# LSimon95/megatts2

Measured on AMD Instinct MI355X. Metric: mel-frames/sec (whole node), higher is better.
Workload: dtype f32; 1 GPU; C3: B=32/GPU x 1 GPU, Np=70, Tp=431, Tm=431; stages vqpe+mrte+adm+plm+decoder+vocoder; forced durations; weights=synthetic (name-seeded), parallelism=dp1 (utterance shards, one RCCL all-gather of mels per step)

## Files before the change

### include/megatts2_hip.h

```cpp
#ifndef MEGATTS2_HIP_H
#define MEGATTS2_HIP_H

#include <stddef.h>
#include <stdint.h>

#ifdef __cplusplus
extern "C" {
#endif

typedef struct mt2_model mt2_model;

typedef struct mt2_config {
    int32_t mel_bins, mrte_hidden, mrte_kernel, mrte_stride, mrte_n_layer, mrte_n_stack, mrte_n_block;
    int32_t content_ff_dim, content_n_heads, content_n_layers, phone_vocab;
    int32_t vq_mel_bins, vq_stride, vq_hidden, vq_kernel, vq_n_layers, vq_n_stacks, vq_n_blocks, vq_bins, vq_dim;
    int32_t dec_kernel, dec_hidden, dec_n_stack, dec_n_block;
    int32_t plm_layers, plm_heads, plm_vq_dim, plm_tc_dim, plm_bins;
    int32_t adm_layers, adm_heads, adm_emb_dim, adm_tc_dim, adm_tc_emb_dim;
    int32_t hg_in_dim, hg_init_channels, hg_n_up, hg_up_rates[8], hg_up_kernels[8];
    int32_t hg_n_res, hg_res_kernels[4], hg_res_dilations[4][3];
    float hg_slope;
    int32_t max_positions;
    int32_t hg_inference_padding;
    int32_t hg_reflect_pad;
// ... 243 lines not shown
} mt2_attn_desc;
int mt2_op_attention_desc(void* stream, const mt2_attn_desc* d);
int mt2_attention_route(const mt2_attn_desc* d, int32_t* err, int32_t* kernel, int32_t* tmpl, int32_t* launch, long long* lds);
int mt2_gemm_trace_begin(mt2_model* m);
int mt2_gemm_trace_end(mt2_model* m, int cap, const char** names, int64_t* launches, double* flops, double* ms);
int mt2_gemm_trace_shapes(mt2_model* m, char* buf, int cap, int top);
int mt2_gemm_config_count(void);
const char* mt2_gemm_config_name(int idx);
int mt2_gemm_route(int M, int N, int K, int taps, int dil, int groups, int pro_act, int operands, int misaligned, int force_cfg,
                   int x3h, int* err, int* cfg, int* variant, long long* lds, int* planes);
int mt2_conv_pair_route(int R, int C, int taps, int dil, int flags, int pair_fuse, int x3h, int* err, long long* lds, int* grid,
                        int* block, int* bm, int* bmo);
int mt2_op_conv_pair(void* stream, const float* X, int ldx, int R, int C, int taps, int dil, float slope, const void* Wh1,
                     const float* inv1, const float* bias1, const void* Wh2, const float* inv2, const float* bias2,
                     const int32_t* valid, float* Y, int ldy, int pair_fuse, int32_t* range_flag);
int mt2_op_gemm_x3h_ln(void* stream, const float* X, int ldx, int Rx, int a_mul, int shift0, const float* W, const void* W3,
                       const void* Wh, const float* wh_inv, const float* bias, const float* R, int ldr, float* C, int ldc, int M, int N,
                       int K, int epi_act, int force_cfg, float* stat_out, int32_t* stat_nt, int32_t* stat_w, const float* ln_stat,
                       int ln_nt, int ln_w, const float* ln_s, float ln_eps);
int mt2_bench_gemm(void* stream, int M, int N, int K, int taps, int dil, int flags, int force_cfg, int iters,
                   int w_copies, float* avg_ms, char* cfg_name, int cfg_name_cap, double* sustained_ghz);

#ifdef __cplusplus
}
#endif
#endif
```

### megatts2_amd/csrc/capi.inc

```

#include <climits>

namespace mt2 {
extern thread_local std::string g_last_error;
void finalize_model(mt2_model& m);
}

using namespace mt2;

#define MT2_API_BEGIN try {
#define MT2_API_END                                 \
    ::CallScope::verdict_of_open_call();            \
    return 0;                                       \
    }                                               \
    catch (const std::exception& e) {               \
        g_last_error = e.what();                    \
        return -1;                                  \
    }                                               \
    catch (...) {                                   \
        g_last_error = "unknown error";             \
        return -1;                                  \
    }

enum Need { NEED_G = 1, NEED_ADM = 2, NEED_PLM = 4, NEED_VOC = 8 };
// ... 257 lines not shown
    if (n == "t_x6_128") return &m->opts.t_x6_128;
    if (n == "t_x3h_128") return &m->opts.t_x3h_128;
    if (n == "x3h") return &m->opts.x3h;
    if (n == "x6_ks") return &m->opts.x6_ks;
    if (n == "voc_streams") return &m->opts.voc_streams;
    if (n == "ldr_prio") return &m->opts.ldr_prio;
    if (n == "skinny_rows") return &m->opts.skinny_rows;
    if (n == "skinny_nw") return &m->opts.skinny_nw;
    if (n == "skinny_pairs") return &m->opts.skinny_pairs;
    if (n == "attn_lds_min") return &m->opts.attn_lds_min;
    if (n == "attn_x6_min") return &m->opts.attn_x6_min;
    if (n == "ln_pairs_adm") return &m->opts.ln_pairs_adm;
    if (n == "ln_pairs_maxm") return &m->opts.ln_pairs_maxm;
    if (n == "a_planes") return &m->opts.a_planes;
    if (n == "pair_fuse") return &m->opts.pair_fuse;
    return nullptr;
}
static bool* option_flag(mt2_model* m, const std::string& n) {
    if (n == "splitk") return &m->opts.splitk;
    if (n == "stage_markers") return &m->opts.markers;
    if (n == "win_conv") return &m->opts.win_conv;
    if (n == "x6_conv") return &m->opts.x6_conv;
    if (n == "x6_gemm") return &m->opts.x6_gemm;
    if (n == "skinny_tm") return &m->opts.skinny_tm;
    if (n == "ldr64") return &m->opts.ldr64;
    return nullptr;
}
int mt2_set_option(mt2_model* m, const char* name, int value) {
    MT2_API_BEGIN
    MT2_REQUIRE(m != nullptr && name != nullptr, "null argument");
// ... 844 lines not shown
    return 0;
}
int mt2_op_conv_pair(void* stream, const float* X, int ldx, int R, int C, int taps, int dil, float slope, const void* Wh1,
                     const float* inv1, const float* bias1, const void* Wh2, const float* inv2, const float* bias2,
                     const int32_t* valid, float* Y, int ldy, int pair_fuse, int32_t* range_flag) {
    MT2_API_BEGIN
    PairP p{};
    p.X = X; p.ldx = ldx; p.R = R; p.C = C; p.taps = taps; p.dil = dil; p.slope = slope;
    p.Wh1 = Wh1; p.inv1 = inv1; p.bias1 = bias1; p.Wh2 = Wh2; p.inv2 = inv2; p.bias2 = bias2;
    p.wh_ldb = 4ll * (((long long)taps * C + 31) / 32 * 32);
    p.valid = valid; p.Y = Y; p.ldy = ldy;
    EngineOpts o;
    o.pair_fuse = pair_fuse;
    o.x3h_flag = range_flag;
    MT2_HIP(launch_conv_pair(p, (hipStream_t)stream, &o));
    MT2_API_END
}

int mt2_op_gemm(void* stream, const float* X, int ldx, int Rx, const int32_t* rowbase, int a_mul, int shift0,
                int taps, int dil, int Cin, const float* W, int ldw, const float* bias, const float* R, int ldr,
                const int32_t* valid, float* C, int ldc, int M, int N, int pro_act, float pro_slope, int epi_act,
                float out_scale, int force_cfg) {
    MT2_API_BEGIN
    GemmP p{};
    p.X = X; p.ldx = ldx; p.Rx = Rx; p.rowbase = rowbase; p.a_mul = a_mul ? a_mul : 1; p.shift0 = shift0;
    p.taps = taps; p.dil = dil; p.Cin = Cin; p.W = W; p.ldw = ldw; p.bias = bias; p.R = R; p.ldr = ldr;
    p.valid = valid; p.C = C; p.ldc = ldc; p.M = M; p.N = N; p.K = taps * Cin; p.groups = 1;
    p.pro_act = pro_act; p.pro_slope = pro_slope; p.epi_act = epi_act; p.out_scale = out_scale;
    EngineOpts o;
    o.force_cfg = force_cfg;
// ... 531 lines not shown
```

### megatts2_amd/csrc/gemm_x3h.hip

```cpp
#include "gemm_common.h"

#include <atomic>

#ifndef MT2_X3H_ABLATE
#define MT2_X3H_ABLATE 0
#endif
#define MT2_ABL_NOINGEST (MT2_X3H_ABLATE == 2 || MT2_X3H_ABLATE == 5 || MT2_X3H_ABLATE == 6 || MT2_X3H_ABLATE == 7)
#define MT2_ABL_NOSPLIT (MT2_X3H_ABLATE == 3 || MT2_X3H_ABLATE == 5 || MT2_X3H_ABLATE == 6)
#define MT2_ABL_NOBARRIER (MT2_X3H_ABLATE == 6 || MT2_X3H_ABLATE == 7)
#ifdef MT2_X3H_NO_BUFFER_LOADS
#define MT2_BUFFER_LOADS false
#else
#define MT2_BUFFER_LOADS true
#endif

namespace mt2 {

typedef _Float16 f16x8 __attribute__((ext_vector_type(8)));
typedef _Float16 f16x2 __attribute__((ext_vector_type(2)));
typedef float f32x2 __attribute__((ext_vector_type(2)));
typedef unsigned u32x4 __attribute__((ext_vector_type(4)));

constexpr float kX3hLoScale = 2048.0f, kX3hLoInv = 1.0f / 2048.0f, kX3hMaxIn = 65504.0f;

// ... 1376 lines not shown
    const EngineOpts& o = opts ? *opts : kDefaults;
    const PairRoute r = conv_pair_route(p_in, o);
    if (r.err != hipSuccess || r.grid == 0) return r.err;
    const PairTile& c = kPairTiles[r.tile];
    PairP p = p_in;
    p.x3h_flag = o.x3h_flag;
    p.ldr_prio = o.ldr_prio;
    const size_t lds_attr = c.ring + (size_t)(p.C / 32) * ((c.bm + 64 + 7) & ~7) * BK * sizeof(float);
    const hipError_t e = dyn_lds_once(g_pair_attr_done[r.tile], reinterpret_cast<const void*>(c.fn), lds_attr);
    if (e != hipSuccess) return e;
    if (opts) opts->last_cfg = "x3hpair";
    hipLaunchKernelGGL(c.fn, dim3(r.grid), dim3(r.block), r.lds, s, p);
    return hipGetLastError();
}


#define MT2_X3H_LDR(IDX_, BM_, BN_, WM_, WN_, NL_, NST_)                                                                    \
    { IDX_, BM_, BN_, (WM_* WN_ + NL_) * 64, (size_t)NST_ * ((size_t)BM_ * BK * 4 + (size_t)(2 * BN_ / 16) * 1024),         \
      "x3hldr" #BM_ "x" #BN_ "_" #WM_ "x" #WN_ "+" #NL_ "_s" #NST_ "xc",                                                    \
      { gemm_x3h_ldr_kernel<BM_, BN_, WM_, WN_, NL_, NST_, ACT_NONE>, gemm_x3h_ldr_kernel<BM_, BN_, WM_, WN_, NL_, NST_, ACT_RELU>, \
        gemm_x3h_ldr_kernel<BM_, BN_, WM_, WN_, NL_, NST_, ACT_LRELU>, gemm_x3h_ldr_kernel<BM_, BN_, WM_, WN_, NL_, NST_, PRO_APL>, \
        gemm_x3h_ldr_kernel<BM_, BN_, WM_, WN_, NL_, NST_, PRO_LNX> }, PIPE_X3H, 0, 0, (BN_) / (WN_) }
#define MT2_X3H_KS(IDX_, BM_, BN_, WM_, WN_, KS_, NL_, NST_)                                                                \
    { IDX_, BM_, BN_, (WM_* WN_ * KS_ + NL_) * 64, (size_t)KS_ * NST_ * ((size_t)BM_ * BK * 4 + (size_t)(2 * BN_ / 16) * 1024), \
      "x3hks" #BM_ "x" #BN_ "_" #WM_ "x" #WN_ "_k" #KS_ "+" #NL_ "_s" #NST_,                                                \
      { gemm_x3h_ks_kernel<BM_, BN_, WM_, WN_, KS_, NL_, NST_, ACT_NONE>, gemm_x3h_ks_kernel<BM_, BN_, WM_, WN_, KS_, NL_, NST_, ACT_RELU>, \
        gemm_x3h_ks_kernel<BM_, BN_, WM_, WN_, KS_, NL_, NST_, ACT_LRELU>, gemm_x3h_ks_kernel<BM_, BN_, WM_, WN_, KS_, NL_, NST_, PRO_APL>, \
        gemm_x3h_ks_kernel<BM_, BN_, WM_, WN_, KS_, NL_, NST_, PRO_LNX> }, PIPE_X3H, 0, KS_, 32 }
#define MT2_X3H_WIN(IDX_, QS_, BM_, BN_, WM_, WN_, NST_, NL_)                                                               \
    { IDX_, BM_, BN_, (WM_* WN_ + NL_) * 64, (size_t)NST_ * (((2 * BN_ / 16 + NL_ - 1) / NL_) * NL_ * 1024),                  \
// ... 17 lines not shown
```

### megatts2_amd/csrc/model_load.hip

```cpp
#include "mt2_model.h"
#include "x3h_planes.h"

#include <algorithm>
#include <cstring>

namespace mt2 {

thread_local std::string g_last_error;

void check_hip(hipError_t e, const char* what, const char* file, int line) {
    if (e != hipSuccess)
        throw Error(std::string("HIP error ") + hipGetErrorString(e) + " in " + what + " at " + file + ":" +
                    std::to_string(line));
}

Arena::~Arena() {
    for (auto& c : chunks_) (void)hipFree(c.p);
}
void Arena::reset() {
    for (auto& c : chunks_) c.used = 0;
}
void Arena::reserve(size_t bytes) {
    for (auto& c : chunks_)
        if (c.size >= bytes) return;
// ... 380 lines not shown
            for (int ph = 0; ph < hs; ++ph)
                for (int o = 0; o < co; ++o) {
                    float* rl = lo.data() + ((size_t)ph * co + o) * 2 * ch;
                    float* rh = hi.data() + ((size_t)ph * co + o) * 2 * ch;
                    for (int ci = 0; ci < ch; ++ci) {
                        rl[ci] = W(ci, o, ph + hs + s);
                        rl[ch + ci] = W(ci, o, ph + hs);
                        rh[ci] = W(ci, o, ph + s);
                        rh[ch + ci] = W(ci, o, ph);
                    }
                    bias[(size_t)ph * co + o] = b.data[o];
                }
            UpW u;
            u.cin = ch; u.cout = co; u.stride = s;
            u.wlo = L.upload(lo, (size_t)2 * ch); u.whi = L.upload(hi, (size_t)2 * ch); u.bias = L.upload(bias);
            m.hg_up.push_back(u);
            for (int j = 0; j < c.hg_n_res; ++j) {
                ResW r;
                r.k = c.hg_res_kernels[j];
                const std::string rp = "hifigan.resblocks." + std::to_string(i * c.hg_n_res + j);
                for (int n = 0; n < 3; ++n) {
                    r.dil[n] = c.hg_res_dilations[j][n];
                    r.c1[n] = L.conv(rp + ".convs1." + std::to_string(n), co, co, r.k);
                    r.c2[n] = L.conv(rp + ".convs2." + std::to_string(n), co, co, r.k);
                }
                m.hg_res.push_back(r);
            }
            ch = co;
        }
        m.hg_post = L.conv("hifigan.conv_post", 1, ch, 7);
// ... 12 lines not shown
```

### megatts2_amd/csrc/model_stages.hip

```cpp
#include "mt2_model.h"
#include "x3h_planes.h"
#include "gemm_tiles.h"

#include <algorithm>
#include <cmath>
#include <cstring>
#include <numeric>

namespace mt2 {



static RowSet make_rows(const int* lens, int B, int G) {
    RowSet rs;
    rs.B = B; rs.G = G;
    rs.len.assign(lens, lens + B);
    rs.off.resize(B);
    int r = G;
    for (int b = 0; b < B; ++b) {
        MT2_REQUIRE(lens[b] >= 0, "negative utterance length");
        rs.off[b] = r;
        r += lens[b] + G;
        rs.maxlen = std::max(rs.maxlen, lens[b]);
    }
// ... 175 lines not shown
                      bool reflect, float* y, const int* valid) {
    if (w1.k != w2.k || w1.cin != C || w1.cout != C || w2.cin != C || w2.cout != C) return false;
    GemmP g1{}, g2{};
    g1.W = w1.w; g1.taps = w1.k; g1.Cin = C; g1.groups = 1;
    g2.W = w2.w; g2.taps = w2.k; g2.Cin = C; g2.groups = 1;
    attach_planes(c.m, g1);
    attach_planes(c.m, g2);
    if (!g1.W3 || !g2.W3 || g1.wh_ldb != g2.wh_ldb) return false;
    PairP p{};
    p.X = x; p.ldx = C; p.R = R; p.C = C; p.taps = w1.k; p.dil = dil; p.slope = slope;
    p.Wh1 = g1.Wh; p.inv1 = g1.wh_inv; p.bias1 = w1.b;
    p.Wh2 = g2.Wh; p.inv2 = g2.wh_inv; p.bias2 = w2.b;
    p.wh_ldb = g1.wh_ldb ? g1.wh_ldb : 4ll * ((w1.k * C + 31) / 32 * 32);
    p.valid = valid; p.Y = y; p.ldy = C; p.reflect = reflect ? 1 : 0;
    const hipError_t e = launch_conv_pair(p, c.s, &c.m.opts);
    if (e == hipErrorNotSupported) return false;
    MT2_HIP(e);
    return true;
}

static void layernorm(const Ctx& c, const float* x, int ldx, const float* g, const float* b, int M, int C,
                      float* out, int ldo, const int* valid = nullptr, int valid_rows = 0,
                      const float* R1 = nullptr, int ldr1 = 0, int r1_rows = 0, int rows_per_group = 0,
                      int act = ACT_NONE, bool out_planes = false) {
    LnP p{};
    p.x = x; p.ldx = ldx; p.gamma = g; p.beta = b; p.rows_per_group = rows_per_group;
    p.R1 = R1; p.ldr1 = ldr1; p.r1_rows = r1_rows; p.valid = valid; p.valid_rows = valid_rows;
    p.out = out; p.ldo = ldo; p.M = M; p.C = C; p.eps = 1e-5f; p.act = act;
    p.out_planes = out_planes ? 1 : 0; p.x3h_flag = c.m.opts.x3h_flag;
    MT2_HIP(launch_layernorm(p, c.s));
// ... 965 lines not shown
    for (int b = 1; b < M0.B; ++b) min_len = std::min(min_len, M0.len[b]);
    auto halo = [&](const Ctx& cc, float* buf, int width, int G) {
        if (!reflect || G <= 0) return;
        MT2_REQUIRE(2ll * G <= (long long)M0.G * scale, "reflect padding needs a gap of two halos between utterances");
        MT2_REQUIRE((long long)min_len * scale > G, "reflect padding must be smaller than the utterance (as F.pad raises): "
                                                    "utterance too short for the vocoder's reflect-padded convolutions");
        MT2_HIP(launch_fill_reflect(buf, width, width, M0.d_start, M0.d_len, M0.B, scale, G, cc.s));
    };
    float* x = c.ws.get<float>((size_t)R * ch);
    if (reflect) {
        MT2_REQUIRE((cfg.hg_in_dim & 3) == 0, "reflect padding needs a mel width that is a multiple of 4");
        halo(c, const_cast<float*>(xmel), cfg.hg_in_dim, (m.hg_pre.k - 1) / 2);
    }
    conv_same(c, xmel, cfg.hg_in_dim, (int)R, m.hg_pre, x, ch, M0.d_valid);
    const int* valid = M0.d_valid;
    for (int i = 0; i < cfg.hg_n_up; ++i) {
        const UpW& u = m.hg_up[i];
        const int s = u.stride, co = u.cout, hs = s / 2;
        MT2_REQUIRE(R * s < (1ll << 31), "waveform row count exceeds int32");
        float* up = c.ws.get<float>((size_t)R * s * co);
        for (int half = 0; half < 2; ++half) {
            GemmP p{};
            p.X = x; p.ldx = ch; p.Rx = (int)R; p.taps = 2; p.shift0 = half == 0 ? -1 : 0; p.Cin = ch;
            p.W = half == 0 ? u.wlo : u.whi; p.bias = u.bias; p.valid = valid;
            p.C = up + (half == 0 ? 0 : hs * co); p.ldc = s * co; p.M = (int)R; p.N = hs * co;
            p.pro_act = ACT_LRELU; p.pro_slope = slope;
            gemm(c, p);
        }
        int* v2 = c.ws.get<int>((size_t)R * s);
        MT2_HIP(launch_expand_mask(valid, s, v2, R * s, c.s));
        valid = v2;
        R *= s;
        scale *= s;
        ch = co;
        const size_t per = (size_t)R * ch;
        float* rb[3] = {nullptr, nullptr, nullptr};
        MT2_REQUIRE(cfg.hg_n_res == 3, "HiFi-GAN V1 uses three resblocks per stage");
        const int nside = m.opts.voc_streams > 1 ? 2 : 0;
        ensure_aux(m, nside);
        if (reflect) {
            int g0 = 0;
            for (int j = 0; j < 3; ++j) g0 = std::max(g0, (m.hg_res[i * 3 + j].k - 1) / 2 * m.hg_res[i * 3 + j].dil[0]);
            halo(c, up, ch, g0);
        }
        if (nside) {
            MT2_HIP(hipEventRecord(m.ev_fork, c.s));
            m.aux_forked = true;
            for (int j = 0; j < nside; ++j) MT2_HIP(hipStreamWaitEvent(m.aux_streams[j], m.ev_fork, 0));
        }
        for (int j = 0; j < 3; ++j) {
            const ResW& r = m.hg_res[i * 3 + j];
// ... 14 lines not shown
                halo(cj, t1, ch, (r.k - 1) / 2);
                conv_same(cj, t1, ch, (int)R, r.c2[n], out, ch, valid, ACT_NONE, slope, ACT_NONE, h, ch, 1);
                h = out;
            }
        }
        for (int j = 0; j < nside; ++j) {
            MT2_HIP(hipEventRecord(m.ev_join[j], m.aux_streams[j]));
            MT2_HIP(hipStreamWaitEvent(c.s, m.ev_join[j], 0));
        }
        if (!reflect && i + 1 == cfg.hg_n_up && m.hg_post.cout == 1 && (ch & 3) == 0 && ch <= 128 && m.hg_post.k <= 15) {
            float* wav = c.ws.get<float>((size_t)R);
            const hipError_t e = launch_conv_post(rb[0], rb[1], rb[2], 1.0f / 3.0f, R, ch, m.hg_post.k, m.hg_post.w,
                                                  m.hg_post.b, 0.01f, valid, wav, c.s);
            if (e == hipSuccess) return wav;
            if (e != hipErrorNotSupported) MT2_HIP(e);
        }
        x = c.ws.get<float>(per);
        MT2_HIP(launch_avg3(rb[0], rb[1], rb[2], 1.0f / 3.0f, x, (long long)per, c.s));
    }
    float* wav = c.ws.get<float>((size_t)R);
    halo(c, x, ch, (m.hg_post.k - 1) / 2);
    conv_same(c, x, ch, (int)R, m.hg_post, wav, 1, valid, ACT_LRELU, 0.01f, ACT_TANH);
    return wav;
}


static double hz_to_mel_slaney(double f) {
    const double f_sp = 200.0 / 3.0, min_log_hz = 1000.0, min_log_mel = min_log_hz / f_sp, logstep = std::log(6.4) / 27.0;
    return f >= min_log_hz ? min_log_mel + std::log(f / min_log_hz) / logstep : f / f_sp;
}
// ... 609 lines not shown
```

### megatts2_amd/csrc/mt2_kernels.h

```cpp
#pragma once
#include <hip/hip_runtime.h>
#include <stdint.h>

#include <atomic>
#include <vector>

namespace mt2 {

inline hipError_t dyn_lds_once(std::atomic<unsigned long long>& done, const void* fn, size_t bytes) {
    int dev = 0;
    hipError_t e = hipGetDevice(&dev);
    if (e != hipSuccess) return e;
    const unsigned long long bit = 1ull << (dev & 63);
    if (done.load(std::memory_order_acquire) & bit) return hipSuccess;
    e = hipFuncSetAttribute(fn, hipFuncAttributeMaxDynamicSharedMemorySize, (int)bytes);
    if (e != hipSuccess) return e;
    done.fetch_or(bit, std::memory_order_release);
    return hipSuccess;
}

constexpr int kInvalidRow = -(1 << 30);

enum Act : int { ACT_NONE = 0, ACT_RELU = 1, ACT_LRELU = 2, ACT_TANH = 3,
                 ACT_LOGCLAMP = 4 };
// ... 29 lines not shown
    const float* ln_g; const float* ln_b; float ln_eps;
    float* stat_out = nullptr; int stat_nt = 0, stat_w = 0;
    const float* ln_stat = nullptr; int ln_nt = 0, ln_w = 0;
};
struct TraceRec { int cfg; double flops; hipEvent_t e0, e1; int M, N, K, groups; };
struct EngineOpts {
    int force_cfg = -1;
    int t_ks4 = 256, t_ks2 = 640, t32 = 64, t32x32 = 160;
    bool splitk = true;
    int voc_streams = 3;
    bool win_conv = true;
    bool x6_conv = true;
    bool x6_gemm = true;
    int x3h = 15;
    int pair_fuse = 3;
    int* x3h_flag = nullptr;
    int t_x3h_128 = 72;
    int t_x6_256 = 160, t_x6_128 = 72;
    int x6_ks = 4;
    int a_planes = 3;
    bool ldr64 = false;
    int ldr_prio = 3;
    int skinny_rows = 64;
    int attn_lds_min = 640;
    int attn_x6_min = 192;
    bool skinny_tm = true;
    int skinny_pairs = 1;
    int skinny_nw = 16;
    bool markers = false;
    bool trace_on = false;
// ... 12 lines not shown
    const float* X; int ldx;
    int R, C, taps, dil;
    float slope;
    const void* Wh1; const float* inv1; const float* bias1;
    const void* Wh2; const float* inv2; const float* bias2;
    long long wh_ldb;
    const int* valid;
    float* Y; int ldy;
    int reflect = 0;
    int* x3h_flag = nullptr;
    int ldr_prio = 0;
};
struct PairRoute { hipError_t err; int tile; size_t lds; unsigned grid, block; int bm, bmo; };
PairRoute conv_pair_route(const PairP& p, const EngineOpts& o);
hipError_t launch_conv_pair(const PairP& p, hipStream_t s, EngineOpts* o = nullptr);
bool gemm_takes_planes(const GemmP& p, const EngineOpts& o);
bool gemm_writes_planes(const GemmP& p, const EngineOpts& o);
bool gemm_skinny_eligible(const GemmP& p, int max_rows);
hipError_t launch_gemm_skinny(const GemmP& p, hipStream_t s);
bool gemm_skinny_tm_eligible(const GemmP& p, int max_rows);
hipError_t launch_gemm_skinny_tm(const GemmP& p, hipStream_t s);
hipError_t launch_tile_major(const float* W, int N, int K, float* out, hipStream_t s);
int gemm_num_configs();
const char* gemm_config_name(int idx);
int gemm_trace_collect(EngineOpts& o, int cap, const char** names, int64_t* launches, double* flops, double* ms);
int gemm_trace_shapes(EngineOpts& o, char* buf, int cap, int top);

struct LnP {
    const float* x; int ldx;
    const float* gamma; const float* beta; int rows_per_group;
// ... 204 lines not shown
```

### megatts2_amd/csrc/mt2_model.h

```cpp
#pragma once
#include "../../include/megatts2_hip.h"
#include "mt2_kernels.h"

#include <map>
#include <mutex>
#include <stdexcept>
#include <string>
#include <vector>

namespace mt2 {

struct Error : std::runtime_error {
    using std::runtime_error::runtime_error;
};
void check_hip(hipError_t e, const char* what, const char* file, int line);
#define MT2_HIP(x) ::mt2::check_hip((x), #x, __FILE__, __LINE__)
#define MT2_REQUIRE(cond, msg)                                                                   \
    do {                                                                                         \
        if (!(cond)) throw ::mt2::Error(std::string(msg) + " [" #cond "] at " __FILE__ ":" +     \
                                        std::to_string(__LINE__));                               \
    } while (0)

class Arena {
  public:
// ... 55 lines not shown
struct TmRange { const float* base; size_t n; int K; const float* tm; };
struct StackW {
    float *w = nullptr, *b = nullptr, *g = nullptr, *be = nullptr;
    int C = 0, k = 0, nstack = 0, nblock = 0, groups = 0;
    size_t idx(int s, int blk) const { return (size_t)(s * nblock + blk) * groups; }
};
struct EncLayerW {
    float *ln1g, *ln1b, *ln2g, *ln2b, *wqkv, *bqkv, *wo, *bo, *ff0w, *ff0b, *ff1w, *ff1b;
    float *wqkv_l = nullptr, *sqkv = nullptr, *cqkv = nullptr, *ff0_l = nullptr, *sff0 = nullptr, *cff0 = nullptr;
};
struct EncW {
    std::vector<EncLayerW> layers;
    int d = 0, ff = 0, heads = 0;
    bool conv_ff = false;
};
struct UpW { float *wlo, *whi, *bias; int cin, cout, stride; };
struct ResW { ConvW c1[3], c2[3]; int k; int dil[3]; };

struct StageTimer {
    std::vector<std::string> names;
    std::vector<hipEvent_t> ev;
};

}

struct mt2_model {
    mt2_config cfg{};
    bool finalized = false;
    bool has_g = false, has_adm = false, has_plm = false;
    std::map<std::string, mt2::HostTensor> host;
    std::vector<void*> dev_allocs;
// ... 61 lines not shown
```

### megatts2_amd/runtime.py

```python
from __future__ import annotations

import ctypes as C
import math
import os
from typing import Dict, Optional, Sequence

import numpy as np

from . import config as cfgmod
from . import sampling as sampmod

_LIB = None
MAX_POSITIONS = 8192

MT2_RUN_PLM, MT2_RUN_VOCODER, MT2_SKIP_ADM, MT2_PROMPT_VQPE = 1, 2, 4, 8
ACT_NONE, ACT_RELU, ACT_LRELU, ACT_TANH = 0, 1, 2, 3
ACT_LOGCLAMP = 4
MT2_RESAMPLE_NORMALIZE = 1
TRIM_FRAME, TRIM_HOP = 2048, 512
F0_FRAME, F0_WINDOW, F0_MAX_LAG = 1024, 768, 256
DTW_MAX_LEN, DTW_DIR_COLS = 4096, 16


class NativeError(RuntimeError):
# ... 940 lines not shown
    if out is None:
        out = torch.empty(R, Cc, device=X.device, dtype=torch.float32)
    flag = torch.zeros(4, device=X.device, dtype=torch.int32)
    _check(lib.mt2_op_conv_pair(_stream(), _ptr(X), X.shape[1], R, Cc, taps, dil, C.c_float(slope), _ptr(p1), _ptr(i1), _ptr(b1),
                                _ptr(p2), _ptr(i2), _ptr(b2), _ptr(valid), _ptr(out), out.shape[1], pair_fuse, _ptr(flag)))
    return (out, int(flag[0].item())) if want_flag else out


def op_conv_pair_route(R, Cn, taps, dil, flags=0, pair_fuse=7, x3h=15):
    err, lds, grid, block, bm, bmo = C.c_int(0), C.c_longlong(0), C.c_int(0), C.c_int(0), C.c_int(0), C.c_int(0)
    load_library().mt2_conv_pair_route(R, Cn, taps, dil, flags, pair_fuse, x3h, C.byref(err), C.byref(lds), C.byref(grid), C.byref(block),
                                       C.byref(bm), C.byref(bmo))
    return {"err": err.value, "lds": lds.value, "grid": grid.value, "block": block.value, "bm": bm.value, "bmo": bmo.value}


def op_gemm_x6_ln(X, W, bias=None, R=None, M=None, a_mul=1, shift0=0, epi_act=ACT_NONE, force_cfg=-1, want_stats=False,
                  ln=None, eps=1e-5, x3h=False):
    import torch
    lib = load_library()
    K, N = X.shape[1], W.shape[0]
    M = M or X.shape[0]
    dev = X.device
    out = torch.empty(M, N, device=dev, dtype=torch.float32)
    stat = torch.zeros(M, 32, 2, device=dev, dtype=torch.float32) if want_stats else None
    nt, pw = C.c_int32(0), C.c_int32(0)
    ln_stat, ln_nt, ln_w, ln_s = None, 0, 0, None
    if ln is not None:
        gamma, beta, pairs, ln_w = ln
        Wd = W.double().cpu()
        Wl = (W.cpu() * gamma.cpu()[None, :]).to(torch.float32)
# ... 356 lines not shown
```

Baseline: 83780 mel-frames/s.

## Fuse resblock average with stride-2 vocoder upsample into one x3h kernel

Adds an up_mrf kernel that reads the three multi-receptive-field resblock outputs, averages and applies leaky ReLU while staging the window in LDS, then runs both transposed-conv phases for stride-2 upsampling as a single split-f16 MFMA GEMM. The kernel uses concatenated lo/hi weights and a dedicated loader-wave ring. This removes the separate avg3 pass and its intermediate buffer, and replaces two GEMM launches with one. It adds a complex new kernel with f16 split precision and range-flag checks. It falls back to the old path when the shape is unsupported.

After: 84760 mel-frames/s, median of 6. 1.01x the previous value.

```diff
diff --git a/include/megatts2_hip.h b/include/megatts2_hip.h
--- a/include/megatts2_hip.h
+++ b/include/megatts2_hip.h
@@ -281,6 +281,11 @@
 int mt2_op_conv_pair(void* stream, const float* X, int ldx, int R, int C, int taps, int dil, float slope, const void* Wh1,
                      const float* inv1, const float* bias1, const void* Wh2, const float* inv2, const float* bias2,
                      const int32_t* valid, float* Y, int ldy, int pair_fuse, int32_t* range_flag);
+int mt2_up_mrf_route(int R, int ch, int stride, int flags, int up_fuse, int x3h, int off, int* err, long long* lds, int* grid, int* block,
+                     int* bm);
+int mt2_op_up_mrf(void* stream, const float* X0, const float* X1, const float* X2, int ldx, int R, int ch, float scale, float slope,
+                  const void* Wh, const float* inv, const float* bias, const int32_t* valid, float* Y, int ldy, int up_fuse,
+                  int32_t* range_flag);
 int mt2_op_gemm_x3h_ln(void* stream, const float* X, int ldx, int Rx, int a_mul, int shift0, const float* W, const void* W3,
                        const void* Wh, const float* wh_inv, const float* bias, const float* R, int ldr, float* C, int ldc, int M, int N,
                        int K, int epi_act, int force_cfg, float* stat_out, int32_t* stat_nt, int32_t* stat_w, const float* ln_stat,
diff --git a/megatts2_amd/csrc/capi.inc b/megatts2_amd/csrc/capi.inc
--- a/megatts2_amd/csrc/capi.inc
+++ b/megatts2_amd/csrc/capi.inc
@@ -295,6 +295,7 @@
     if (n == "ln_pairs_maxm") return &m->opts.ln_pairs_maxm;
     if (n == "a_planes") return &m->opts.a_planes;
     if (n == "pair_fuse") return &m->opts.pair_fuse;
+    if (n == "up_fuse") return &m->opts.up_fuse;
     return nullptr;
 }
 static bool* option_flag(mt2_model* m, const std::string& n) {
@@ -1169,6 +1170,49 @@
     o.pair_fuse = pair_fuse;
     o.x3h_flag = range_flag;
     MT2_HIP(launch_conv_pair(p, (hipStream_t)stream, &o));
+    MT2_API_END
+}
+
+int mt2_up_mrf_route(int R, int ch, int stride, int flags, int up_fuse, int x3h, int off, int* err, long long* lds, int* grid, int* block,
+                     int* bm) {
+    alignas(128) static char dummy[8 * 128];
+    UpMrfP p{};
+    p.X0 = (const float*)dummy; p.X1 = (flags & 32) ? nullptr : (const float*)(dummy + 128); p.X2 = (const float*)(dummy + 256);
+    p.ldx = ch; p.R = R; p.ch = ch; p.stride = stride; p.scale = 1.0f / 3.0f; p.slope = 0.1f;
+    if (!(flags & 1)) { p.Wh = dummy + 384 + ((flags & 8) ? 16 : 0); p.inv = (const float*)(dummy + 512); }
+    p.bias = (const float*)(dummy + 640 + ((flags & 128) ? 4 : 0));
+    p.wh_ldb = 8ll * ch;
+    p.Y = (float*)(dummy + 768 + ((flags & 4) ? 4 : 0)); p.ldy = ch;
+    if ((flags & 2) && R > 0) p.ldx = (int)((((1ll << 31) / 4 + R - 1) / R + 3) & ~3ll);
+    if (flags & 16) p.ldx = ch + 2;
+    if (flags & 64) p.ldy = ch - 4;
+    EngineOpts o;
+    o.up_fuse = up_fuse;
+    o.x3h = x3h;
+    if (off & 1) o.win_conv = false;
+    if (off & 2) o.x6_conv = false;
+    if (off & 4) o.force_cfg = 0;
+    if (off & 8) o.ldr64 = true;
+    const UpMrfRoute r = up_mrf_route(p, o);
+    if (err) *err = (int)r.err;
+    if (lds) *lds = (long long)r.lds;
+    if (grid) *grid = (int)r.grid;
+    if (block) *block = (int)r.block;
+    if (bm) *bm = r.bm;
+    return 0;
+}
+int mt2_op_up_mrf(void* stream, const float* X0, const float* X1, const float* X2, int ldx, int R, int ch, float scale, float slope,
+                  const void* Wh, const float* inv, const float* bias, const int32_t* valid, float* Y, int ldy, int up_fuse,
+                  int32_t* range_flag) {
+    MT2_API_BEGIN
+    UpMrfP p{};
+    p.X0 = X0; p.X1 = X1; p.X2 = X2; p.ldx = ldx; p.R = R; p.ch = ch; p.stride = 2; p.scale = scale; p.slope = slope;
+    p.Wh = Wh; p.inv = inv; p.bias = bias; p.wh_ldb = 8ll * ch;
+    p.valid = valid; p.Y = Y; p.ldy = ldy;
+    EngineOpts o;
+    o.up_fuse = up_fuse;
+    o.x3h_flag = range_flag;
+    MT2_HIP(launch_up_mrf(p, (hipStream_t)stream, &o));
     MT2_API_END
 }
 
diff --git a/megatts2_amd/csrc/gemm_x3h.hip b/megatts2_amd/csrc/gemm_x3h.hip
--- a/megatts2_amd/csrc/gemm_x3h.hip
+++ b/megatts2_amd/csrc/gemm_x3h.hip
@@ -1414,6 +1414,328 @@
     return hipGetLastError();
 }
 
+template <int QS, int BM, int BN, int WGM, int WGN, int NST, int NL>
+__global__ __launch_bounds__((WGM * WGN + NL) * 64) void up_mrf_x3h_kernel(UpMrfP p) {
+    constexpr int NW = WGM * WGN;
+    constexpr int WTM = BM / WGM, WTN = BN / WGN;
+    constexpr int TM = WTM / 32, TN = WTN / 32;
+    constexpr int NPH = WGN == 2 ? 1 : 2;
+    constexpr int CO = BN / 2;
+    constexpr int BPIECES = BN / 8;
+    constexpr int NI = NL;
+    constexpr int B_IT = (BPIECES + NI - 1) / NI;
+    constexpr int STAGE_B = B_IT * NI * 1024;
+    constexpr int NT = (NW + NL) * 64;
+    constexpr int WR = BM + 2, WRp = (WR + 7) & ~7;
+    constexpr int NTASK = QS * WRp * 4, MAXT = (NTASK + NT - 1) / NT;
+    constexpr int NK = 2 * QS;
+    static_assert(NL > 0 && WTM % 32 == 0 && WTN % 32 == 0 && NST >= 3 && (NST - 2) * B_IT < 64 && BN == 32 * QS, "config");
+    static_assert((WGN == 2 && WTN == CO) || (WGN == 1 && TN == 2), "a wave's columns are one phase, or one 32-column tile per phase");
+    static_assert(NK >= NST - 1 && QS >= 2, "the ring's first stages are whole chunks of this launch");
+
+    extern __shared__ __attribute__((aligned(16))) float smem[];
+    const int tid = threadIdx.x, lane = tid & 63;
+    const int wave_all = __builtin_amdgcn_readfirstlane(tid >> 6);
+    const bool loader = wave_all >= NW;
+    const int wave = loader ? wave_all - NW : wave_all;
+    const int wm = wave / WGN, wn = wave % WGN;
+    char* ring = reinterpret_cast<char*>(smem);
+    float* win = smem + NST * STAGE_B / 4;
+
+    const int ntm = (p.R + BM - 1) / BM;
+    const int bid = blockIdx.x;
+    const int xcd = bid & 7, qq = ntm >> 3, rr = ntm & 7;
+    const int tile = (xcd < rr ? xcd * (qq + 1) : rr * (qq + 1) + (xcd - rr) * qq) + (bid >> 3);
+    const int m0 = tile * BM;
+    const int row_first = m0 - 1;
+    const int ldx = p.ldx, Rx = p.R;
+
+    {
+        const float* __restrict__ X = p.X0;
+        const long long zoff_x = (const float*)g_zero16 - X;
+        const int lrow = lane >> 3;
+        constexpr int ppq = WRp >> 3, pieces = QS * ppq;
+        for (int pc = wave_all; pc < pieces; pc += NW + NL) {
+            const int q = pc / ppq, r8 = pc - q * ppq;
+            const int row = r8 * 8 + lrow;
+            const int grow = row_first + row;
+            const int slot = (lane & 7) ^ ((row >> 1) & 7);
+            const bool ok = (row < WR) & ((unsigned)grow < (unsigned)Rx);
+            const long long off = ok ? (long long)grow * ldx + q * 32 + slot * 4 : zoff_x;
+            __builtin_amdgcn_global_load_lds((const __attribute__((address_space(1))) void*)(X + off),
+                                             (__attribute__((address_space(3))) void*)(win + (q * WRp + r8 * 8) * 32), 16, 0, 0);
+        }
+    }
+    f32x4 xb[MAXT][2], xc[MAXT][2];
+#pragma unroll
+    for (int u = 0; u < MAXT; ++u) {
+        const int t = tid + u * NT;
+        const int tt = t < NTASK ? t : 0;
+        const int rbk = tt >> 2, j = tt & 3;
+        const int q = rbk / WRp, row = rbk - q * WRp;
+        const int grow = row_first + row;
+        const bool ok = (t < NTASK) & (row < WR) & ((unsigned)grow < (unsigned)Rx);
+        const long long off = (long long)grow * ldx + q * 32 + j * 8;
+        const float* s1 = ok ? p.X1 + off : (const float*)g_zero16;
+        const float* s2 = ok ? p.X2 + off : (const float*)g_zero16;
+        const int o2 = ok ? 4 : 0;
+        xb[u][0] = *reinterpret_cast<const f32x4*>(s1); xb[u][1] = *reinterpret_cast<const f32x4*>(s1 + o2);
+        xc[u][0] = *reinterpret_cast<const f32x4*>(s2); xc[u][1] = *reinterpret_cast<const f32x4*>(s2 + o2);
+    }
+    constexpr unsigned kOut = 0x80000000u;
+    unsigned vob[B_IT];
+#pragma unroll
+    for (int j = 0; j < B_IT; ++j) {
+        const int pc = j * NI + wave;
+        const int n = pc * 8 + (lane >> 3);
+        const int sl = (lane & 7) ^ ((n >> 1) & 7);
+        vob[j] = (pc < BPIECES && n < BN) ? (unsigned)(n * (int)p.wh_ldb + sl * 16) : kOut;
+    }
+    const __amdgpu_buffer_rsrc_t rs_w = __builtin_amdgcn_make_buffer_rsrc(const_cast<char*>(reinterpret_cast<const char*>(p.Wh)), 0, (int)kOut, 0x00020000);
+    auto issue = [&](int c, int st) __attribute__((always_inline)) {
+        char* Bs = ring + st * STAGE_B + wave * 1024;
+#pragma unroll
+        for (int j = 0; j < B_IT; ++j)
+            __builtin_amdgcn_raw_ptr_buffer_load_lds(rs_w, (__attribute__((address_space(3))) void*)(Bs + j * NI * 1024), 16, (int)vob[j], c * 128, 0, 0);
+    };
+    if (loader) {
+        loader_priority(p.ldr_prio);
+#pragma unroll
+        for (int st = 0; st < NST - 1; ++st) issue(st, st);
+        wait_vmcnt<(NST - 1) * B_IT>();
+    } else {
+        wait_vmcnt<0>();
+    }
+    float amax = 0.0f;
+    {
+        const unsigned lds_w = (unsigned)(unsigned long long)(__attribute__((address_space(3))) float*)win;
+        f32x4 in[MAXT][2];
+        __builtin_amdgcn_s_barrier();
+        asm volatile("" ::: "memory");
+#pragma unroll
+        for (int u = 0; u < MAXT; ++u) {
+            const int t = tid + u * NT;
+            const int tt = t < NTASK ? t : 0;
+            const int rbk = tt >> 2, j = tt & 3;
+            const int swz = ((rbk % WRp) >> 1) & 7;
+            const unsigned base = lds_w + (unsigned)rbk * 128;
+            in[u][0] = lds_read_b128(base + (unsigned)(((2 * j) ^ swz) * 16));
+            in[u][1] = lds_read_b128(base + (unsigned)(((2 * j + 1) ^ swz) * 16));
+        }
+        asm volatile("s_waitcnt lgkmcnt(0)" ::: "memory");
+#pragma unroll
+        for (int u = 0; u < MAXT; ++u) asm volatile("" : "+v"(in[u][0]), "+v"(in[u][1]));
+        __builtin_amdgcn_s_barrier();
+        asm volatile("" ::: "memory");
+        const float scale = p.scale, slope = p.slope;
+#pragma unroll
+        for (int u = 0; u < MAXT; ++u) {
+            const int t = tid + u * NT;
+            if (t < NTASK) {
+                const int rbk = t >> 2, j = t & 3;
+                const int swz = ((rbk % WRp) >> 1) & 7;
+                f32x4 mv[2];
+#pragma unroll
+                for (int h = 0; h < 2; ++h)
+#pragma unroll
+                    for (int e = 0; e < 4; ++e) mv[h][e] = ((in[u][h][e] + xb[u][h][e]) + xc[u][h][e]) * scale;
+                u32x4 ph, pl;
+                split2_f16<ACT_LRELU>(mv[0], mv[1], slope, ph, pl, amax);
+                char* dst = reinterpret_cast<char*>(win) + (size_t)rbk * 128;
+                *reinterpret_cast<u32x4*>(dst + ((j ^ swz) * 16)) = ph;
+                *reinterpret_cast<u32x4*>(dst + (((4 + j) ^ swz) * 16)) = pl;
+            }
+        }
+        asm volatile("s_waitcnt lgkmcnt(0)" ::: "memory");
+    }
+    if (p.x3h_flag != nullptr && __builtin_amdgcn_ballot_w64(amax >= kX3hMaxIn) != 0ull && lane == 0) atomicOr(p.x3h_flag, 1);
+    if (loader) {
+        for (int c = 0; c < NK; ++c) {
+            if (c == 0) { if (NST - 2 < NK) wait_vmcnt<(NST - 2) * B_IT>(); else wait_vmcnt<0>(); }
+            else if (c + NST - 3 < NK) wait_vmcnt<(NST - 3) * B_IT>();
+            else wait_vmcnt<0>();
+            __builtin_amdgcn_s_barrier();
+            if (c >= 1 && c + NST - 2 < NK) issue(c + NST - 2, (c + NST - 2) % NST);
+        }
+        return;
+    }
+    float inv_s[TN], bs[TN];
+#pragma unroll
+    for (int j = 0; j < TN; ++j) {
+        const int n = wn * WTN + j * 32 + (lane & 31);
+        inv_s[j] = p.inv[n];
+        bs[j] = p.bias ? p.bias[n & (CO - 1)] : 0.0f;
+    }
+    f32x16 acc[TM][TN], acl[TM][TN];
+#pragma unroll
+    for (int i = 0; i < TM; ++i)
+#pragma unroll
+        for (int j = 0; j < TN; ++j)
+#pragma unroll
+            for (int e = 0; e < 16; ++e) { acc[i][j][e] = 0.0f; acl[i][j][e] = 0.0f; }
+
+    const int half = lane >> 5;
+    const unsigned lds_ring = (unsigned)(unsigned long long)(__attribute__((address_space(3))) char*)ring;
+    const unsigned lds_win = (unsigned)(unsigned long long)(__attribute__((address_space(3))) float*)win;
+    const int nrow = wn * WTN + (lane & 31);
+    const unsigned b_lane = lds_ring + nrow * 128;
+    const int swzb = (nrow >> 1) & 7;
+    unsigned koffb[2][2];
+#pragma unroll
+    for (int b = 0; b < 2; ++b) {
+        koffb[b][0] = (unsigned)(((b * 2 + half) ^ swzb) * 16);
+        koffb[b][1] = (unsigned)(((4 + b * 2 + half) ^ swzb) * 16);
+    }
+    const int arow0 = wm * WTM + (lane & 31) + (NPH == 1 ? wn : 0);
+    constexpr int N1 = 2 * NPH * TM + 2 * TN;
+    static_assert(N1 <= 15, "lgkmcnt is four bits wide");
+    u32x4 ra[2][NPH][TM][2];
+    u32x4 rb[2][2][TN];
+    auto fetch_a = [&](int b, int q, int arow) __attribute__((always_inline)) {
+#pragma unroll
+        for (int ph = 0; ph < NPH; ++ph) {
+            const int row = arow + ph;
+            const int swza = (row >> 1) & 7;
+            const unsigned sa = lds_win + (unsigned)((q * WRp + row) * BK) * 4;
+            const unsigned vh = sa + (unsigned)(((b * 2 + half) ^ swza) * 16), vl = sa + (unsigned)(((4 + b * 2 + half) ^ swza) * 16);
+            static_for(std::make_integer_sequence<int, TM>{}, [&](auto ic) {
+                constexpr int i = decltype(ic)::value;
+                ra[b][ph][i][0] = __builtin_bit_cast(u32x4, lds_read_b128_imm<i * 32 * BK * 4>(vh));
+                ra[b][ph][i][1] = __builtin_bit_cast(u32x4, lds_read_b128_imm<i * 32 * BK * 4>(vl));
+            });
+        }
+    };
+    auto fetch_b = [&](int b, unsigned sb) __attribute__((always_inline)) {
+        const unsigned vb0 = sb + koffb[b][0], vb1 = sb + koffb[b][1];
+        static_for(std::make_integer_sequence<int, TN>{}, [&](auto ic) {
+            constexpr int j = decltype(ic)::value;
+            rb[b][0][j] = __builtin_bit_cast(u32x4, lds_read_b128_imm<j * 32 * 128>(vb0));
+            rb[b][1][j] = __builtin_bit_cast(u32x4, lds_read_b128_imm<j * 32 * 128>(vb1));
+        });
+    };
+    auto tie_set = [&](int b) __attribute__((always_inline)) {
+#pragma unroll
+        for (int ph = 0; ph < NPH; ++ph)
+#pragma unroll
+            for (int i = 0; i < TM; ++i) asm volatile("" : "+v"(ra[b][ph][i][0]), "+v"(ra[b][ph][i][1]));
+#pragma unroll
+        for (int pl = 0; pl < 2; ++pl)
+#pragma unroll
+            for (int j = 0; j < TN; ++j) asm volatile("" : "+v"(rb[b][pl][j]));
+    };
+    auto products = [&](int b) __attribute__((always_inline)) {
+#pragma unroll
+        for (int i = 0; i < TM; ++i) {
+#pragma unroll
+            for (int j = 0; j < TN; ++j)
+                acl[i][j] = __builtin_amdgcn_mfma_f32_32x32x16_f16(__builtin_bit_cast(f16x8, ra[b][NPH == 1 ? 0 : j][i][0]),
+                                                                   __builtin_bit_cast(f16x8, rb[b][1][j]), acl[i][j], 0, 0, 0);
+#pragma unroll
+            for (int j = 0; j < TN; ++j)
+                acc[i][j] = __builtin_amdgcn_mfma_f32_32x32x16_f16(__builtin_bit_cast(f16x8, ra[b][NPH == 1 ? 0 : j][i][0]),
+                                                                   __builtin_bit_cast(f16x8, rb[b][0][j]), acc[i][j], 0, 0, 0);
+#pragma unroll
+            for (int j = 0; j < TN; ++j)
+                acl[i][j] = __builtin_amdgcn_mfma_f32_32x32x16_f16(__builtin_bit_cast(f16x8, ra[b][NPH == 1 ? 0 : j][i][1]),
+                                                                   __builtin_bit_cast(f16x8, rb[b][0][j]), acl[i][j], 0, 0, 0);
+        }
+    };
+    __builtin_amdgcn_s_barrier();
+    asm volatile("" ::: "memory");
+    fetch_a(0, 0, arow0); fetch_b(0, b_lane); fetch_a(1, 0, arow0); fetch_b(1, b_lane);
+    __builtin_amdgcn_sched_barrier(0);
+    int stn = 1 % NST, tapn = 0, qn = 1;
+    auto chunk = [&](auto last_c) __attribute__((always_inline)) {
+        constexpr bool last = decltype(last_c)::value;
+        const int arow = arow0 + tapn;
+        const unsigned sb = b_lane + (unsigned)stn * STAGE_B;
+#pragma unroll
+        for (int b = 0; b < 2; ++b) {
+            if (last && b == 1) asm volatile("s_waitcnt lgkmcnt(0)" ::: "memory");
+            else asm volatile("s_waitcnt lgkmcnt(%0)" :: "n"(N1) : "memory");
+            tie_set(b);
+            __builtin_amdgcn_sched_barrier(0);
+            products(b);
+            __builtin_amdgcn_sched_barrier(0);
+            if constexpr (!last) {
+                if (b == 0) {
+                    __builtin_amdgcn_s_barrier();
+                    asm volatile("" ::: "memory");
+                }
+                fetch_a(b, qn, arow);
+                fetch_b(b, sb);
+                __builtin_amdgcn_sched_barrier(0);
+            }
+        }
+        stn = stn + 1 == NST ? 0 : stn + 1;
+        if (++qn == QS) { qn = 0; ++tapn; }
+    };
+    for (int c = 0; c + 1 < NK; ++c) chunk(std::false_type{});
+    chunk(std::true_type{});
+#pragma unroll
+    for (int i = 0; i < TM; ++i)
+#pragma unroll
+        for (int j = 0; j < TN; ++j)
+#pragma unroll
+            for (int e = 0; e < 16; ++e) {
+                float v = __builtin_fmaf(acl[i][j][e], kX3hLoInv, acc[i][j][e]) * inv_s[j];
+                asm volatile("" : "+v"(v));
+                acc[i][j][e] = v + bs[j];
+            }
+    GemmP e{};
+    e.valid = p.valid; e.C = p.Y; e.ldc = p.ldy; e.M = p.R; e.N = BN; e.epi_act = ACT_NONE; e.out_scale = 1.0f;
+    epilogue_t4<TM, TN>(e, acc, 0, m0 + wm * WTM, wn * WTN, lane);
+}
+
+typedef void (*UpMrfKernel)(UpMrfP);
+struct UpMrfTile { int ch, bm, threads; size_t ring; UpMrfKernel fn; };
+#define MT2_UPMRF_TILE(QS_, BM_, BN_, WM_, WN_, NST_, NL_)                                                                   \
+    { BN_, BM_, (WM_* WN_ + NL_) * 64, (size_t)NST_ * (((2 * BN_ / 16 + NL_ - 1) / NL_) * NL_ * 1024),                        \
+      up_mrf_x3h_kernel<QS_, BM_, BN_, WM_, WN_, NST_, NL_> }
+static const UpMrfTile kUpMrfTiles[2] = { MT2_UPMRF_TILE(2, 256, 64, 8, 1, 4, 4), MT2_UPMRF_TILE(4, 128, 128, 4, 2, 3, 4) };
+
+UpMrfRoute up_mrf_route(const UpMrfP& p, const EngineOpts& o) {
+    UpMrfRoute r{hipSuccess, -1, 0, 0, 0, 0};
+    const auto fail = [&r](hipError_t e) { r.err = e; r.tile = -1; r.lds = 0; r.grid = r.block = 0; r.bm = 0; return r; };
+    if (p.R <= 0) return r;
+    const int t = p.ch == 64 ? 0 : (p.ch == 128 ? 1 : -1);
+    if (t < 0 || p.stride != 2 || !((o.up_fuse >> t) & 1)) return fail(hipErrorNotSupported);
+    if (!o.win_conv || !o.x6_conv || !(o.x3h & 4) || o.force_cfg >= 0 || o.ldr64) return fail(hipErrorNotSupported);
+    if (!p.Wh || !p.inv) return fail(hipErrorNotSupported);
+    const long long two_g = 1ll << 31;
+    if ((long long)p.R * p.ldx * 4 >= two_g || (long long)p.R * p.ldy * 4 >= two_g || (long long)p.ch * p.wh_ldb >= two_g - 1)
+        return fail(hipErrorNotSupported);
+    if (!p.X0 || !p.X1 || !p.X2 || !p.Y || p.ldx < p.ch || p.ldy < p.ch || p.wh_ldb < 8ll * p.ch) return fail(hipErrorInvalidValue);
+    if (((p.ldx | p.ldy) & 3) || (p.wh_ldb & 127) || ((unsigned long long)p.Wh & 127) ||
+        (((unsigned long long)p.X0 | (unsigned long long)p.X1 | (unsigned long long)p.X2 | (unsigned long long)p.Y | (unsigned long long)p.bias) & 15))
+        return fail(hipErrorNotSupported);
+    const UpMrfTile& c = kUpMrfTiles[t];
+    r.tile = t;
+    r.bm = c.bm;
+    r.lds = c.ring + (size_t)(p.ch / 32) * ((c.bm + 2 + 7) & ~7) * BK * sizeof(float);
+    r.grid = (unsigned)((p.R + c.bm - 1) / c.bm);
+    r.block = (unsigned)c.threads;
+    return r;
+}
+
+static std::atomic<unsigned long long> g_upmrf_attr_done[2];
+
+hipError_t launch_up_mrf(const UpMrfP& p_in, hipStream_t s, EngineOpts* opts) {
+    static const EngineOpts kDefaults;
+    const EngineOpts& o = opts ? *opts : kDefaults;
+    const UpMrfRoute r = up_mrf_route(p_in, o);
+    if (r.err != hipSuccess || r.grid == 0) return r.err;
+    const UpMrfTile& c = kUpMrfTiles[r.tile];
+    UpMrfP p = p_in;
+    p.x3h_flag = o.x3h_flag;
+    p.ldr_prio = o.ldr_prio;
+    const hipError_t e = dyn_lds_once(g_upmrf_attr_done[r.tile], reinterpret_cast<const void*>(c.fn), r.lds);
+    if (e != hipSuccess) return e;
+    if (opts) opts->last_cfg = "x3hupmrf";
+    hipLaunchKernelGGL(c.fn, dim3(r.grid), dim3(r.block), r.lds, s, p);
+    return hipGetLastError();
+}
+
 
 #define MT2_X3H_LDR(IDX_, BM_, BN_, WM_, WN_, NL_, NST_)                                                                    \
     { IDX_, BM_, BN_, (WM_* WN_ + NL_) * 64, (size_t)NST_ * ((size_t)BM_ * BK * 4 + (size_t)(2 * BN_ / 16) * 1024),         \
diff --git a/megatts2_amd/csrc/model_load.hip b/megatts2_amd/csrc/model_load.hip
--- a/megatts2_amd/csrc/model_load.hip
+++ b/megatts2_amd/csrc/model_load.hip
@@ -418,6 +418,11 @@
             UpW u;
             u.cin = ch; u.cout = co; u.stride = s;
             u.wlo = L.upload(lo, (size_t)2 * ch); u.whi = L.upload(hi, (size_t)2 * ch); u.bias = L.upload(bias);
+            if (s == 2) {
+                std::vector<float> cat(lo);
+                cat.insert(cat.end(), hi.begin(), hi.end());
+                u.wcat = L.upload(cat, (size_t)2 * ch);
+            }
             m.hg_up.push_back(u);
             for (int j = 0; j < c.hg_n_res; ++j) {
                 ResW r;
diff --git a/megatts2_amd/csrc/model_stages.hip b/megatts2_amd/csrc/model_stages.hip
--- a/megatts2_amd/csrc/model_stages.hip
+++ b/megatts2_amd/csrc/model_stages.hip
@@ -213,6 +213,22 @@
     p.wh_ldb = g1.wh_ldb ? g1.wh_ldb : 4ll * ((w1.k * C + 31) / 32 * 32);
     p.valid = valid; p.Y = y; p.ldy = C; p.reflect = reflect ? 1 : 0;
     const hipError_t e = launch_conv_pair(p, c.s, &c.m.opts);
+    if (e == hipErrorNotSupported) return false;
+    MT2_HIP(e);
+    return true;
+}
+
+static bool up_mrf(const Ctx& c, const float* const* rb, int ch, int R, const UpW& u, float slope, float* up, const int* valid) {
+    if (!u.wcat || u.cin != ch || u.cout * 2 != ch) return false;
+    GemmP g{};
+    g.W = u.wcat; g.taps = 2; g.Cin = ch; g.groups = 1;
+    attach_planes(c.m, g);
+    UpMrfP p{};
+    p.X0 = rb[0]; p.X1 = rb[1]; p.X2 = rb[2]; p.ldx = ch; p.R = R; p.ch = ch; p.stride = u.stride;
+    p.scale = 1.0f / 3.0f; p.slope = slope;
+    p.Wh = g.Wh; p.inv = g.wh_inv; p.bias = u.bias; p.wh_ldb = g.wh_ldb ? g.wh_ldb : 8ll * ch;
+    p.valid = valid; p.Y = up; p.ldy = 2 * u.cout;
+    const hipError_t e = launch_up_mrf(p, c.s, &c.m.opts);
     if (e == hipErrorNotSupported) return false;
     MT2_HIP(e);
     return true;
@@ -1208,12 +1224,23 @@
     }
     conv_same(c, xmel, cfg.hg_in_dim, (int)R, m.hg_pre, x, ch, M0.d_valid);
     const int* valid = M0.d_valid;
+    const float* const* mrf = nullptr;
+    float* rb[3] = {nullptr, nullptr, nullptr};
     for (int i = 0; i < cfg.hg_n_up; ++i) {
         const UpW& u = m.hg_up[i];
         const int s = u.stride, co = u.cout, hs = s / 2;
         MT2_REQUIRE(R * s < (1ll << 31), "waveform row count exceeds int32");
         float* up = c.ws.get<float>((size_t)R * s * co);
-        for (int half = 0; half < 2; ++half) {
+        bool fused = false;
+        if (mrf) {
+            fused = m.opts.up_fuse && up_mrf(c, mrf, ch, (int)R, u, slope, up, valid);
+            if (!fused) {
+                x = c.ws.get<float>((size_t)R * ch);
+                MT2_HIP(launch_avg3(mrf[0], mrf[1], mrf[2], 1.0f / 3.0f, x, R * ch, c.s));
+            }
+            mrf = nullptr;
+        }
+        for (int half = 0; half < 2 && !fused; ++half) {
             GemmP p{};
             p.X = x; p.ldx = ch; p.Rx = (int)R; p.taps = 2; p.shift0 = half == 0 ? -1 : 0; p.Cin = ch;
             p.W = half == 0 ? u.wlo : u.whi; p.bias = u.bias; p.valid = valid;
@@ -1228,7 +1255,6 @@
         scale *= s;
         ch = co;
         const size_t per = (size_t)R * ch;
-        float* rb[3] = {nullptr, nullptr, nullptr};
         MT2_REQUIRE(cfg.hg_n_res == 3, "HiFi-GAN V1 uses three resblocks per stage");
         const int nside = m.opts.voc_streams > 1 ? 2 : 0;
         ensure_aux(m, nside);
@@ -1273,6 +1299,10 @@
                                                   m.hg_post.b, 0.01f, valid, wav, c.s);
             if (e == hipSuccess) return wav;
             if (e != hipErrorNotSupported) MT2_HIP(e);
+        }
+        if (i + 1 < cfg.hg_n_up) {
+            mrf = rb;
+            continue;
         }
         x = c.ws.get<float>(per);
         MT2_HIP(launch_avg3(rb[0], rb[1], rb[2], 1.0f / 3.0f, x, (long long)per, c.s));
diff --git a/megatts2_amd/csrc/mt2_kernels.h b/megatts2_amd/csrc/mt2_kernels.h
--- a/megatts2_amd/csrc/mt2_kernels.h
+++ b/megatts2_amd/csrc/mt2_kernels.h
@@ -67,6 +67,7 @@
     bool x6_gemm = true;
     int x3h = 15;
     int pair_fuse = 3;
+    int up_fuse = 3;
     int* x3h_flag = nullptr;
     int t_x3h_128 = 72;
     int t_x6_256 = 160, t_x6_128 = 72;
@@ -109,6 +110,19 @@
 struct PairRoute { hipError_t err; int tile; size_t lds; unsigned grid, block; int bm, bmo; };
 PairRoute conv_pair_route(const PairP& p, const EngineOpts& o);
 hipError_t launch_conv_pair(const PairP& p, hipStream_t s, EngineOpts* o = nullptr);
+struct UpMrfP {
+    const float* X0; const float* X1; const float* X2; int ldx;
+    int R, ch, stride;
+    float scale, slope;
+    const void* Wh; const float* inv; const float* bias; long long wh_ldb;
+    const int* valid;
+    float* Y; int ldy;
+    int* x3h_flag = nullptr;
+    int ldr_prio = 0;
+};
+struct UpMrfRoute { hipError_t err; int tile; size_t lds; unsigned grid, block; int bm; };
+UpMrfRoute up_mrf_route(const UpMrfP& p, const EngineOpts& o);
+hipError_t launch_up_mrf(const UpMrfP& p, hipStream_t s, EngineOpts* o = nullptr);
 bool gemm_takes_planes(const GemmP& p, const EngineOpts& o);
 bool gemm_writes_planes(const GemmP& p, const EngineOpts& o);
 bool gemm_skinny_eligible(const GemmP& p, int max_rows);
diff --git a/megatts2_amd/csrc/mt2_model.h b/megatts2_amd/csrc/mt2_model.h
--- a/megatts2_amd/csrc/mt2_model.h
+++ b/megatts2_amd/csrc/mt2_model.h
@@ -93,7 +93,8 @@
     int d = 0, ff = 0, heads = 0;
     bool conv_ff = false;
 };
-struct UpW { float *wlo, *whi, *bias; int cin, cout, stride; };
+struct UpW { float *wlo, *whi, *bias; int cin, cout, stride;
+             float* wcat = nullptr; };
 struct ResW { ConvW c1[3], c2[3]; int k; int dil[3]; };
 
 struct StageTimer {
diff --git a/megatts2_amd/runtime.py b/megatts2_amd/runtime.py
--- a/megatts2_amd/runtime.py
+++ b/megatts2_amd/runtime.py
@@ -978,6 +978,28 @@
     return {"err": err.value, "lds": lds.value, "grid": grid.value, "block": block.value, "bm": bm.value, "bmo": bmo.value}
 
 
+def op_up_mrf(X0, X1, X2, Wcat, bias, slope, scale=1.0 / 3.0, valid=None, channels=None, out=None, up_fuse=3, want_flag=False):
+    import torch
+    lib = load_library()
+    ch = channels or X0.shape[1]
+    R = X0.shape[0]
+    assert X1.shape == X0.shape and X2.shape == X0.shape
+    ph, inv = (t.to(X0.device) for t in split_f16x2_rows(Wcat))
+    if out is None:
+        out = torch.empty(R, ch, device=X0.device, dtype=torch.float32)
+    flag = torch.zeros(4, device=X0.device, dtype=torch.int32)
+    _check(lib.mt2_op_up_mrf(_stream(), _ptr(X0), _ptr(X1), _ptr(X2), X0.shape[1], R, ch, C.c_float(scale), C.c_float(slope), _ptr(ph),
+                             _ptr(inv), _ptr(bias), _ptr(valid), _ptr(out), out.shape[1], up_fuse, _ptr(flag)))
+    return (out, int(flag[0].item())) if want_flag else out
+
+
+def op_up_mrf_route(R, ch, stride=2, flags=0, up_fuse=3, x3h=15, off=0):
+    err, lds, grid, block, bm = C.c_int(0), C.c_longlong(0), C.c_int(0), C.c_int(0), C.c_int(0)
+    load_library().mt2_up_mrf_route(R, ch, stride, flags, up_fuse, x3h, off, C.byref(err), C.byref(lds), C.byref(grid), C.byref(block),
+                                    C.byref(bm))
+    return {"err": err.value, "lds": lds.value, "grid": grid.value, "block": block.value, "bm": bm.value}
+
+
 def op_gemm_x6_ln(X, W, bias=None, R=None, M=None, a_mul=1, shift0=0, epi_act=ACT_NONE, force_cfg=-1, want_stats=False,
                   ln=None, eps=1e-5, x3h=False):
     import torch
```
